# LepistaBioinformatics/blutils

Measured on AMD Instinct MI355X. Metric: Mqueries/sec consensus (synthetic outfmt-6 hit table), higher is better.
Workload: dtype i32/u32

## Files before the change

### blutils_amd/csrc/consensus_kernel.hip

```cpp

#if defined(__HIP_DEVICE_COMPILE__) && !defined(__gfx950__)
#error "consensus_kernel.hip is written for gfx950"
#endif

#include <hip/hip_runtime.h>

#include <climits>
#include <cstdint>
#include <type_traits>

#include "blu_internal.h"

namespace blu {

#define WAVE 64

constexpr int BLOCK_A = 768;
constexpr int BLU_WAVES_PER_SIMD = 3;
constexpr int BLOCK_N = 1024;
constexpr int BLU_N_WAVES_PER_SIMD = 4;
constexpr int BLOCK_F = 704;
constexpr int LIST_CAP = 208;
constexpr int LIST_CAP_RING = 248;
constexpr int LIST_CAP_F64 = 232;
// ... 681 lines not shown
                else { m[0] = wave_max_i32(m[0]); m[1] = wave_max_i32(m[1]); }
                uint32_t c[2], slot[2], tot[2], tmask[2];
#pragma unroll
                for (int hf = 0; hf < 2; ++hf) {
                    c[hf] = 0; tmask[hf] = 0;
#pragma unroll
                    for (int r = 0; r < 4; ++r) { const bool t = left[hf] > r && bs[hf][r] == m[hf]; tmask[hf] |= (uint32_t)t << r; c[hf] += (uint32_t)t; }
                    uint32_t in = c[hf];
                    in += (uint32_t)dpp<0x111>((int)in);
                    in += (uint32_t)dpp<0x112>((int)in);
                    in += (uint32_t)dpp<0x114>((int)in);
                    in += (uint32_t)dpp<0x118>((int)in);
                    const uint32_t k0 = (uint32_t)rl((int)in, 15), k1 = (uint32_t)rl((int)in, 31), k2 = (uint32_t)rl((int)in, 47), k3 = (uint32_t)rl((int)in, 63);
                    tot[hf] = k0 + k1 + k2 + k3;
                    slot[hf] = (row16 == 0 ? 0u : (row16 == 1 ? k0 : (row16 == 2 ? k0 + k1 : k0 + k1 + k2))) + in - c[hf];
                }
                const uint32_t gk = tot[0] + tot[1];
                const bool fits = fill + gk <= CAP;
                if (lane == 0) {
                    if (halves) L.meta[qi] = fits ? (fill | (gk << 16)) : META_SLOW;
                    else {
                        L.meta[qs[0]] = fits ? (fill | (tot[0] << 16)) : META_SLOW;
                        if (qs[1] < 64u) L.meta[qs[1]] = fits ? ((fill + tot[0]) | (tot[1] << 16)) : META_SLOW;
                    }
                }
                if (!fits) {
                    uint64_t rest = long_mask;
                    while (rest) { const uint32_t qn = (uint32_t)__builtin_ctzll(rest); rest &= rest - 1; if (lane == 0) L.meta[qn] = META_SLOW; }
                    break;
                }
                {
#pragma unroll
                    for (int hf = 0; hf < 2; ++hf) {
                        if (tot[hf] == 0) continue;
                        StepRegs S;
                        fetch_rest(S, voff[hf], tmask[hf]);
                        uint32_t idx = fill + (hf ? tot[0] : 0u) + slot[hf];
#pragma unroll
                        for (int r = 0; r < 4; ++r) {
                            if ((tmask[hf] >> r) & 1u) {
                                put_entry(idx, S, r, ro[hf] + sub4 + r);
                                ++idx;
                            }
                        }
                    }
                    fill += gk;
                }
            }
        };
        auto phase1_flat = [&]() {
            if constexpr (!RING) {
            constexpr uint32_t UR = FLAT_ROWS, MAXS = FLAT_STEPS, DEPTH = FLAT_DEPTH;
            static_assert(UR == 8u, "two 16-byte loads per lane");
            static_assert(FLAT_SEG >= MAX_TASK_SEG, "the flat pass takes every segment of the task");
            static_assert(DEPTH <= MAXS && MAXS * WAVE >= FLAT_SEG / UR, "a query's units fit one round");
            const uint32_t rows = L.seg[lane].y;
            const uint32_t nunit = (rows + UR - 1u) / UR;
            uint32_t incl = nunit;
            incl += (uint32_t)dpp<0x111>((int)incl);
            incl += (uint32_t)dpp<0x112>((int)incl);
            incl += (uint32_t)dpp<0x114>((int)incl);
            incl += (uint32_t)dpp<0x118>((int)incl);
            const uint32_t t0 = (uint32_t)rl((int)incl, 15), t1 = (uint32_t)rl((int)incl, 31), t2 = (uint32_t)rl((int)incl, 47);
            const uint32_t r16 = (uint32_t)lane >> 4;
            incl += r16 == 0 ? 0u : (r16 == 1 ? t0 : (r16 == 2 ? t0 + t1 : t0 + t1 + t2));
            const uint32_t q_end = incl, q_begin = incl - nunit;
            const uint64_t out_m = __ballot(rows != 0u && q_end > MAXS * WAVE);
            const uint32_t q_lim = out_m ? (uint32_t)__builtin_ctzll(out_m) : WAVE;
            const uint32_t total = q_lim < WAVE ? (uint32_t)rl((int)q_begin, (int)q_lim) : (uint32_t)rl((int)q_end, WAVE - 1);
            const uint32_t ns = (total + WAVE - 1u) / WAVE;
            L.qs[lane] = q_begin;
            L.qm[lane] = INT_MIN;
            L.qk[lane] = 0u;
            if (rows != 0u) L.meta[lane] = META_SLOW;
            __builtin_amdgcn_fence(__ATOMIC_RELEASE, "workgroup");
            __builtin_amdgcn_wave_barrier();
            __builtin_amdgcn_fence(__ATOMIC_ACQUIRE, "workgroup");
            auto issue = [&](const uint32_t st, u32x4& lo4, u32x4& hi4, uint32_t& um) {
                um = 0u;
                uint32_t voff = 0xFFFFFFF0u;
                int left = 0;
                if (st < ns) {
                    const uint32_t g = st * WAVE + (uint32_t)lane;
                    uint32_t q = 0;
#pragma unroll
                    for (uint32_t sp = 32; sp; sp >>= 1) { const uint32_t c = q + sp; if (L.qs[c] <= g) q = c; }
                    const uint2 sg = L.seg[q];
                    const uint32_t oq = g - L.qs[q];
                    left = g < total ? (int)sg.y - (int)(UR * oq) : 0;
                    if (left > 0) { voff = (sg.x + UR * oq) * 4u; um = q | (oq << 6) | (umin((uint32_t)left, UR) << 12); }
                }
                lo4 = __builtin_amdgcn_raw_buffer_load_b128(rs_bs, voff, 0, STREAM_AUX);
                hi4 = __builtin_amdgcn_raw_buffer_load_b128(rs_bs, left > 4 ? voff + 16u : 0xFFFFFFF0u, 0, STREAM_AUX);
            };
            u32x4 ba[DEPTH], bb[DEPTH];
            uint32_t um[MAXS];
            int lmx[MAXS];
#pragma unroll
            for (uint32_t st = 0; st < MAXS; ++st) { um[st] = 0u; lmx[st] = INT_MIN; }
#pragma unroll
            for (uint32_t st = 0; st < DEPTH; ++st) issue(st, ba[st], bb[st], um[st]);
#pragma unroll
            for (uint32_t st = 0; st < MAXS; ++st) {
                if (st >= ns) break;
                const u32x4 va = ba[st % DEPTH], vb = bb[st % DEPTH];
                const uint32_t left = (um[st] >> 12) & 15u;
                const uint32_t v[8] = {va.x, va.y, va.z, va.w, vb.x, vb.y, vb.z, vb.w};
                int bsv[UR], mx = INT_MIN;
#pragma unroll
                for (uint32_t r = 0; r < UR; ++r) { bsv[r] = left > r ? (int)v[r] : INT_MIN; mx = imax(mx, bsv[r]); }
                uint32_t lmask = 0;
#pragma unroll
                for (uint32_t r = 0; r < UR; ++r) lmask |= (uint32_t)(left > r && bsv[r] == mx) << r;
                um[st] |= lmask << 16;
                lmx[st] = mx;
                if (left) atomicMax(&L.qm[um[st] & 63u], mx);
                if (st + DEPTH < MAXS) issue(st + DEPTH, ba[st % DEPTH], bb[st % DEPTH], um[st + DEPTH]);
            }
            __builtin_amdgcn_fence(__ATOMIC_RELEASE, "workgroup");
            __builtin_amdgcn_wave_barrier();
            __builtin_amdgcn_fence(__ATOMIC_ACQUIRE, "workgroup");
            uint32_t running = fill, q_cut = q_lim;
#pragma unroll
            for (uint32_t st = 0; st < MAXS; ++st) {
                if (st >= ns) break;
                const uint32_t q = um[st] & 63u, oq = (um[st] >> 6) & 63u;
                const bool have = ((um[st] >> 12) & 15u) != 0u;
                const int M = L.qm[q];
                const uint32_t tmask = (have && lmx[st] == M) ? (um[st] >> 16) & 0xFFu : 0u;
                const uint32_t c = (uint32_t)__builtin_popcount(tmask);
                uint32_t in2 = c;
                in2 += (uint32_t)dpp<0x111>((int)in2);
                in2 += (uint32_t)dpp<0x112>((int)in2);
                in2 += (uint32_t)dpp<0x114>((int)in2);
                in2 += (uint32_t)dpp<0x118>((int)in2);
                const uint32_t k0 = (uint32_t)rl((int)in2, 15), k1 = (uint32_t)rl((int)in2, 31), k2 = (uint32_t)rl((int)in2, 47), k3 = (uint32_t)rl((int)in2, 63);
                in2 += r16 == 0 ? 0u : (r16 == 1 ? k0 : (r16 == 2 ? k0 + k1 : k0 + k1 + k2));
                const uint32_t idx0 = running + in2 - c;
                if (have && oq == 0u) L.meta[q] = META_SLOW | idx0;
                if (c) atomicAdd(&L.qk[q], c);
                const bool over = have && idx0 + c > CAP;
                const uint64_t over_m = __ballot(over);
                const bool room = !over && c != 0u && (over_m == 0ull || (uint32_t)lane < (uint32_t)__builtin_ctzll(over_m));
                if (room) L.rec[idx0] = make_uint4(__builtin_bitreverse32(tmask), L.seg[q].x + UR * oq, UR * oq, 0u);
                if (over_m) { q_cut = (uint32_t)rl((int)q, __builtin_ctzll(over_m)); break; }
                running += k0 + k1 + k2 + k3;
            }
            __builtin_amdgcn_fence(__ATOMIC_RELEASE, "workgroup");
            __builtin_amdgcn_wave_barrier();
            __builtin_amdgcn_fence(__ATOMIC_ACQUIRE, "workgroup");
            const uint32_t m = L.meta[lane];
            if (rows != 0u && (uint32_t)lane < q_cut) L.meta[lane] = (m & 0xFFFFu) | (L.qk[lane] << 16);
            fill = q_cut < q_lim ? (L.meta[q_cut] & 0xFFFFu) : running;
            if (q_cut < WAVE) stop_q = q_cut;
            }
        };
        auto ring_mark_landed = [&](const uint32_t upto) {
            const uint32_t m0 = (ring_landed + RING_CHUNKS - 1u) & ~(RING_CHUNKS - 1u);
            if (m0 < upto) {
                if ((uint32_t)lane < RING_PAD) L.ring[RING_ROWS + lane] = L.ring[lane];
                __builtin_amdgcn_fence(__ATOMIC_RELEASE, "workgroup");
                __builtin_amdgcn_wave_barrier();
                __builtin_amdgcn_fence(__ATOMIC_ACQUIRE, "workgroup");
            }
            ring_landed = upto;
        };
        auto ring_refill = [&]() {
            if (ring_head < ring_tail) { ring_head = ring_tail; if (ring_landed < ring_tail) ring_landed = ring_tail; }
            const uint32_t lim = ring_end < ring_tail + RING_CHUNKS ? ring_end : ring_tail + RING_CHUNKS;
            if (ring_head < lim) { ring_dma_run(rs_ring, ring_c0, ring_head, lim); ring_head = lim; }
        };
        auto phase1_scan = [&](const auto rpl_c, const auto full_c, const uint32_t LPQ) {
            constexpr uint32_t RPL = decltype(rpl_c)::value;
            constexpr bool FULL = decltype(full_c)::value;
            static_assert(RPL <= RING_PAD && RPL <= 32u, "rows per lane");
            const uint32_t QPS = WAVE / LPQ;
            const uint32_t grp = (uint32_t)lane / LPQ, sub = ((uint32_t)lane & (LPQ - 1u)) * RPL, row16 = (uint32_t)lane >> 4;
            {
                const uint32_t cs = (uint32_t)((vbase + (uint32_t)rl((int)seg_x, (int)first_q)) >> 8);
                if (cs < ring_tail) { wait_vmcnt(0u); ring_head = ring_landed = ring_tail = cs; }
            }
            for (uint32_t qb = first_q / QPS * QPS; qb < nq; qb += QPS) {
                const uint32_t r_lo = (uint32_t)rl((int)seg_x, (int)(qb < first_q ? first_q : qb));
                const uint32_t qn = qb + QPS;
                const uint32_t r_hi = qn < nq ? (uint32_t)rl((int)seg_x, (int)qn) : task_nrows;
                ring_tail = (uint32_t)((vbase + r_lo) >> 8);
                ring_refill();
                if (r_hi > r_lo) {
                    const uint32_t need = (uint32_t)((vbase + r_hi - 1u) >> 8);
                    if (need >= ring_landed) { wait_vmcnt(ring_head - 1u - need); ring_mark_landed(need + 1u); }
                }
                const uint32_t qi = qb + grp;
                const uint2 sg = L.seg[qi];
                const int left0 = (sg.y > short_seg ? 0 : (int)sg.y) - (int)sub;
                const uint32_t over = (FULL && left0 > 0 && left0 < (int)RPL) ? RPL - (uint32_t)left0 : 0u;
                const uint32_t sub_e = sub - over;
                const int left = FULL ? (left0 > 0 ? (int)RPL : 0) : left0;
                const uint32_t row0 = sg.x + sub_e;
                const uint32_t a = ((uint32_t)vbase + sg.x + sub_e) & RING_MASK;
                int b[RPL];
#pragma unroll
                for (uint32_t i = 0; i < RPL; ++i) b[i] = (int)L.ring[a + i];
                asm volatile("s_waitcnt lgkmcnt(0)" ::: "memory");
#pragma unroll
                for (uint32_t i = 0; i < RPL; ++i) asm volatile("" : "+v"(b[i]));
                if (r_hi > r_lo) { ring_tail = (uint32_t)((vbase + r_hi) >> 8); ring_refill(); }
                int M = INT_MIN;
                if constexpr (FULL) {
#pragma unroll
                    for (uint32_t i = 0; i < RPL; ++i) M = imax(M, b[i]);
                    M = left > 0 ? M : INT_MIN;
                } else {
#pragma unroll
                    for (uint32_t i = 0; i < RPL; ++i) { b[i] = (int)i < left ? b[i] : INT_MIN; M = imax(M, b[i]); }
                }
                if (LPQ >= 2) M = imax(M, dpp<0xB1>(M));
                if (LPQ >= 4) M = imax(M, dpp<0x4E>(M));
                if (LPQ >= 8) M = imax(M, dpp<0x141>(M));
                if (LPQ >= 16) M = imax(M, dpp<0x140>(M));
                uint32_t mask = tie_mask<RPL>(b, M);
                mask = left > 0 ? mask : 0u;
                if constexpr (FULL) mask &= 0xFFFFFFFFu >> (32u - RPL + over);
                const uint32_t c = (uint32_t)__builtin_popcount(mask);
                uint32_t incl = c;
                incl += (uint32_t)dpp<0x111>((int)incl);
                incl += (uint32_t)dpp<0x112>((int)incl);
                incl += (uint32_t)dpp<0x114>((int)incl);
                incl += (uint32_t)dpp<0x118>((int)incl);
                const uint32_t k0 = (uint32_t)rl((int)incl, 15), k1 = (uint32_t)rl((int)incl, 31);
                const uint32_t k2 = (uint32_t)rl((int)incl, 47), k3 = (uint32_t)rl((int)incl, 63);
                const bool fits = fill + k0 + k1 + k2 + k3 <= CAP;
                const uint32_t p1 = fill + k0, p2 = p1 + k1, p3 = p2 + k2;
                const uint32_t rbase = row16 == 0 ? fill : (row16 == 1 ? p1 : (row16 == 2 ? p2 : p3));
                uint32_t gk = c;
                if (LPQ >= 2) gk += (uint32_t)dpp<0xB1>((int)gk);
                if (LPQ >= 4) gk += (uint32_t)dpp<0x4E>((int)gk);
                if (LPQ >= 8) gk += (uint32_t)dpp<0x141>((int)gk);
                if (LPQ >= 16) gk += (uint32_t)dpp<0x140>((int)gk);
                if (PID32 && !fits) {
                    __builtin_amdgcn_s_setprio(2);
                    uint64_t BK = 0;
                    uint32_t bacc = 0, bpos = 0, brow = 0, kmin = 0xFFFFFFFFu, pmax = 0, dlo = 0xFFFFFFFFu, dhi = 0, err = 0xFFFFFFFFu;
                    auto reset = [&]() { BK = 0; bacc = 0; bpos = 0; brow = 0; kmin = 0xFFFFFFFFu; pmax = 0; dlo = 0xFFFFFFFFu; dhi = 0; err = 0xFFFFFFFFu; };
                    auto better = [&](const uint64_t K, const uint32_t acc, const uint32_t pos, const uint64_t K2, const uint32_t acc2, const uint32_t pos2) {
                        const bool gt = (K > K2) | ((K == K2) & (acc > acc2)), eq = (K == K2) & (acc == acc2);
                        return STRAT == BLU_RELAXED ? (gt | (eq & (pos > pos2))) : ((!gt & !eq) | (eq & (pos < pos2)));
                    };
                    auto take_record = [&](const u32x4 rec, const uint32_t gp, const bool on) {
                        const uint32_t len = umin(rec.x >> BLU_ROW_BITS, t.max_depth), pos = rec.x & ROW_MASK;
                        const bool unmatched = pos >= t.n_tax, bad = !unmatched && (rec.x >> BLU_ROW_BITS) == 0;
                        const uint32_t e = (gp << 8) | (bad ? (uint32_t)BLU_ST_ERR_BAD_LINEAGE : (uint32_t)BLU_ST_ERR_UNMATCHED_TAXID);
                        err = (on && (unmatched | bad)) ? umin(err, e) : err;
                        const uint32_t pm = rec.y & ((1u << KEY_PID_BITS) - 1u);
                        const uint32_t k1 = (len << KEY_PID_BITS) | pm;
                        const uint64_t K = ((uint64_t)k1 << 32) | (rec.z ^ 0x80000000u);
                        const bool take = on & ((kmin == 0xFFFFFFFFu) | better(K, rec.w, gp, BK, bacc, bpos));
                        BK = take ? K : BK; bacc = take ? rec.w : bacc; bpos = take ? gp : bpos; brow = take ? pos : brow;
                        kmin = on ? umin(kmin, k1) : kmin;
                        const uint32_t pmo = pm | ((!PACKED && rec.y >= (1u << KEY_PID_BITS)) ? 0x80000000u : 0u);
                        pmax = (on && pmo > pmax) ? pmo : pmax;
                        dlo = on ? umin(dlo, pos) : dlo;
                        dhi = (on && pos > dhi) ? pos : dhi;
                    };
                    auto load_record = [&](const uint32_t row, const bool on) {
                        u32x4 r;
                        if (PACKED) r = __builtin_amdgcn_raw_buffer_load_b128(rs_tax, on ? row * 16u : 0xFFFFFFC0u, 0, GATHER_AUX);
                        else {
                            const uint32_t o4 = on ? row * 4u : 0xFFFFFFF0u;
                            r.x = __builtin_amdgcn_raw_buffer_load_b32(rs_tax, o4, 0, GATHER_AUX);
                            r.y = __builtin_amdgcn_raw_buffer_load_b32(rs_pid, o4, 0, GATHER_AUX);
                            r.z = __builtin_amdgcn_raw_buffer_load_b32(rs_aln, o4, 0, GATHER_AUX);
                            r.w = __builtin_amdgcn_raw_buffer_load_b32(rs_acc, o4, 0, GATHER_AUX);
                        }
                        return r;
                    };
                    auto merge = [&](auto ctrl) {
                        constexpr int C = decltype(ctrl)::value;
                        const uint64_t K2 = ((uint64_t)(uint32_t)dpp<C>((int)(uint32_t)(BK >> 32)) << 32) | (uint32_t)dpp<C>((int)(uint32_t)BK);
                        const uint32_t acc2 = (uint32_t)dpp<C>((int)bacc), pos2 = (uint32_t)dpp<C>((int)bpos), row2 = (uint32_t)dpp<C>((int)brow);
                        const uint32_t kmin2 = (uint32_t)dpp<C>((int)kmin);
                        const bool take = (kmin2 != 0xFFFFFFFFu) & ((kmin == 0xFFFFFFFFu) | better(K2, acc2, pos2, BK, bacc, bpos));
                        BK = take ? K2 : BK; bacc = take ? acc2 : bacc; bpos = take ? pos2 : bpos; brow = take ? row2 : brow;
                        kmin = umin(kmin, kmin2);
                        const uint32_t pm2 = (uint32_t)dpp<C>((int)pmax); pmax = pm2 > pmax ? pm2 : pmax;
                        dlo = umin(dlo, (uint32_t)dpp<C>((int)dlo));
                        const uint32_t hi2 = (uint32_t)dpp<C>((int)dhi); dhi = hi2 > dhi ? hi2 : dhi;
                        err = umin(err, (uint32_t)dpp<C>((int)err));
                    };
                    auto deliver = [&](const int src, const bool mine) {
                        const uint32_t f_khi = (uint32_t)__builtin_amdgcn_ds_bpermute(src, (int)(uint32_t)(BK >> 32));
                        const uint32_t f_pos = (uint32_t)__builtin_amdgcn_ds_bpermute(src, (int)bpos), f_row = (uint32_t)__builtin_amdgcn_ds_bpermute(src, (int)brow);
                        const uint32_t f_kmin = (uint32_t)__builtin_amdgcn_ds_bpermute(src, (int)kmin), f_pmax = (uint32_t)__builtin_amdgcn_ds_bpermute(src, (int)pmax);
                        const uint32_t f_lo = (uint32_t)__builtin_amdgcn_ds_bpermute(src, (int)dlo), f_hi = (uint32_t)__builtin_amdgcn_ds_bpermute(src, (int)dhi);
                        const uint32_t f_err = (uint32_t)__builtin_amdgcn_ds_bpermute(src, (int)err);
                        const bool got = mine && f_kmin != 0xFFFFFFFFu;
                        const bool g_ovf = got && (f_pmax & 0x80000000u) != 0u, g_err = got && !g_ovf && f_err != 0xFFFFFFFFu, g_ok = got && !g_ovf && !g_err;
                        dn_flag = g_ovf ? 3u : (g_err ? 2u : (g_ok ? 1u : dn_flag));
                        dn_err = g_err ? (f_err & 0xFFu) : dn_err;
                        dn_pos = g_err ? (f_err >> 8) : dn_pos;
                        if constexpr (PID32) { r_pid = g_ok ? (f_khi & ((1u << KEY_PID_BITS) - 1u)) : r_pid; max_pid = g_ok ? f_pmax : max_pid; }
                        r_len = g_ok ? (f_khi >> KEY_PID_BITS) : r_len; r_row = g_ok ? f_row : r_row; r_pos = g_ok ? f_pos : r_pos;
                        minlen = g_ok ? (f_kmin >> KEY_PID_BITS) : minlen; g_lo = g_ok ? f_lo : g_lo; g_hi = g_ok ? f_hi : g_hi;
                    };
                    const uint32_t tq = (uint32_t)lane;
                    const bool mine = tq >= qb && tq < qn && tq < nq;
                    const uint32_t own0 = (mine ? tq - qb : 0u) * LPQ;
                    if (LPQ <= 4u && BLU_DENSE_Q * (k0 + k1 + k2 + k3) >= r_hi - r_lo) {
                        const uint32_t c4 = (uint32_t)lane & 3u;
#pragma nounroll
                        for (uint32_t g = 0; g < 4u; ++g) {
                            const int own = (int)((16u * g + ((uint32_t)lane >> 2)) * 4u);
                            const uint32_t o_row0 = (uint32_t)__builtin_amdgcn_ds_bpermute(own, (int)row0);
                            const uint32_t o_mask = (uint32_t)__builtin_amdgcn_ds_bpermute(own, (int)mask);
                            const uint32_t o_sub = (uint32_t)__builtin_amdgcn_ds_bpermute(own, (int)sub_e);
                            if (__ballot(o_mask != 0u) == 0ull) continue;
                            reset();
                            constexpr uint32_t NF = PACKED ? 4u : 2u;
#pragma unroll
                            for (uint32_t b0 = 0; b0 < RPL; b0 += 4u * NF) {
                                if (__ballot(((o_mask >> (RPL - 4u * NF - b0)) & ((1u << (4u * NF)) - 1u)) != 0u) == 0ull) continue;
                                u32x4 rq[NF];
#pragma unroll
                                for (uint32_t j = 0; j < NF; ++j) {
                                    const uint32_t i = b0 + 4u * j + c4;
                                    rq[j] = load_record(o_row0 + i, ((o_mask >> (RPL - 1u - i)) & 1u) != 0u);
                                }
#pragma unroll
                                for (uint32_t j = 0; j < NF; ++j) {
                                    const uint32_t i = b0 + 4u * j + c4;
                                    take_record(rq[j], o_sub + i, ((o_mask >> (RPL - 1u - i)) & 1u) != 0u);
                                }
                            }
                            merge(std::integral_constant<int, 0xB1>());
                            merge(std::integral_constant<int, 0x4E>());
                            if (LPQ >= 2) merge(std::integral_constant<int, 0x141>());
                            if (LPQ >= 4) merge(std::integral_constant<int, 0x140>());
                            deliver((int)(((own0 & 15u) * 4u) * 4u), mine && (own0 >> 4) == g);
                        }
                    } else {
                        uint32_t m = mask;
                        while (__ballot(m != 0u)) {
                            u32x4 rq[4];
                            uint32_t gp[4];
#pragma unroll
                            for (int j = 0; j < 4; ++j) {
                                const bool on = m != 0u;
                                const uint32_t hb = on ? 31u - (uint32_t)__builtin_clz(m) : 0u, i = RPL - 1u - hb;
                                m = on ? (m & ~(1u << hb)) : 0u;
                                gp[j] = on ? sub_e + i : 0xFFFFFFFFu;
                                rq[j] = load_record(row0 + i, on);
                            }
#pragma unroll
                            for (int j = 0; j < 4; ++j) take_record(rq[j], gp[j], gp[j] != 0xFFFFFFFFu);
                        }
                        if (LPQ >= 2) merge(std::integral_constant<int, 0xB1>());
                        if (LPQ >= 4) merge(std::integral_constant<int, 0x4E>());
                        if (LPQ >= 8) merge(std::integral_constant<int, 0x141>());
                        if (LPQ >= 16) merge(std::integral_constant<int, 0x140>());
                        deliver((int)(own0 * 4u), mine);
                    }
                    {
                        const uint32_t f_gk = (uint32_t)__builtin_amdgcn_ds_bpermute((int)(own0 * 4u), (int)gk);
                        dn_k = (mine && dn_flag == 1u) ? f_gk : dn_k;
                    }
                    if (sub == 0 && gk != 0u) L.meta[qi] = META_DENSE;
                    __builtin_amdgcn_s_setprio(0);
                    continue;
                }
                uint32_t idx = rbase + incl - c;
                if (!fits) {
                    const uint32_t lane_o = (uint32_t)__builtin_ctzll(__ballot(idx + c > CAP));
                    const uint32_t qo = qb + lane_o / LPQ;
                    const bool taken = qi < qo;
                    if (sub == 0) L.meta[qi] = taken ? (idx | (gk << 16)) : META_SLOW;
                    if (taken && c) { L.rec[idx].x = mask << (32u - RPL); L.rec[idx].y = DESC_WORD1(RPL, row0, sub_e); }
                    fill = (uint32_t)rl((int)idx, (int)((qo - qb) * LPQ));
                    stop_q = qo;
                    wait_vmcnt(0u);
                    ring_head = ring_landed = ring_tail = (uint32_t)((vbase + (uint32_t)rl((int)seg_x, (int)qo)) >> 8);
                    break;
                }
                if (sub == 0) L.meta[qi] = idx | (gk << 16);
                fill = p3 + k3;
                static_assert((RPL == 16u || RPL == 32u) && SHORT_SEG <= 128u, "descriptor word of a lane");
                if (c) { L.rec[idx].x = mask << (32u - RPL); L.rec[idx].y = DESC_WORD1(RPL, row0, sub_e); }
            }
        };
        auto gather_list = [&](auto&& between) {
            constexpr int NG = (CAP + WAVE - 1) / WAVE;
            u32x4 g[NG];
            uint32_t ghi[NG], gpos[NG], ghint[NG];
            uint32_t carry = 0;
#pragma unroll
            for (int u = 0; u < NG; ++u) {
                g[u] = u32x4{0u, 0u, 0u, 0u}; ghi[u] = 0u; gpos[u] = 0u; ghint[u] = 0u;
                if ((uint32_t)u * WAVE >= fill_ring) continue;
                const uint32_t idx = (uint32_t)u * WAVE + (uint32_t)lane;
                const bool valid = idx < fill_ring;
                const uint32_t d0 = L.rec[idx < CAP ? idx : 0u].x;
                int s = (valid && d0 != 0u) ? (int)idx : 0;
                s = imax(s, dpp<0x111>(s));
                s = imax(s, dpp<0x112>(s));
                s = imax(s, dpp<0x114>(s));
                s = imax(s, dpp<0x118>(s));
                s = imax(s, __builtin_amdgcn_update_dpp(0, s, 0x142, 0xA, 0xF, false));
                s = imax(s, __builtin_amdgcn_update_dpp(0, s, 0x143, 0xC, 0xF, false));
                s = imax(s, (int)carry);
                carry = (uint32_t)rl(s, 63);
                const uint4 dd = L.rec[s];
                const uint32_t d0w = dd.x, d = dd.y;
                uint32_t r = idx - (uint32_t)s, x = scan_rpl == 32u ? d0w : d0w >> 16, i = 0;
                if (scan_rpl == 32u) {
                    const uint32_t h = x >> 16, ch = (uint32_t)__builtin_popcount(h);
                    const bool low = r >= ch;
                    r -= low ? ch : 0u; x = low ? (x & 0xFFFFu) : h; i += low ? 16u : 0u;
                }
                {
                    const uint32_t h = x >> 8, ch = (uint32_t)__builtin_popcount(h);
                    const bool low = r >= ch;
                    r -= low ? ch : 0u; x = low ? (x & 0xFFu) : h; i += low ? 8u : 0u;
                }
                {
                    const uint32_t h = x >> 4, ch = (uint32_t)__builtin_popcount(h);
                    const bool low = r >= ch;
                    r -= low ? ch : 0u; x = low ? (x & 0xFu) : h; i += low ? 4u : 0u;
                }
                {
                    const uint32_t h = x >> 2, ch = (uint32_t)__builtin_popcount(h);
                    const bool low = r >= ch;
                    r -= low ? ch : 0u; x = low ? (x & 0x3u) : h; i += low ? 2u : 0u;
                }
                i += (r >= (x >> 1)) ? 1u : 0u;
                const uint32_t row = (RING ? (d >> DESC_SUB_BITS) : d) + i;
                gpos[u] = (RING ? (d & ((1u << DESC_SUB_BITS) - 1u)) : dd.z) + i;
                if (PACKED) g[u] = __builtin_amdgcn_raw_buffer_load_b128(rs_tax, valid ? row * 16u : 0xFFFFFFC0u, 0, GATHER_AUX);
                else if (WIDE) {
                    g[u] = __builtin_amdgcn_raw_buffer_load_b128(rs_tax, valid ? row * 24u : 0xFFFFFFC0u, 0, GATHER_AUX);
                    const u32x2 p = __builtin_amdgcn_raw_buffer_load_b64(rs_tax, valid ? row * 24u + 16u : 0xFFFFFFE0u, 0, GATHER_AUX);
                    ghint[u] = g[u].y;
                    g[u].y = p.x; ghi[u] = p.y;
                } else {
                    const uint32_t o4 = valid ? row * 4u : 0xFFFFFFF0u;
                    g[u].x = __builtin_amdgcn_raw_buffer_load_b32(rs_tax, o4, 0, GATHER_AUX);
                    if (PID32) g[u].y = __builtin_amdgcn_raw_buffer_load_b32(rs_pid, o4, 0, GATHER_AUX);
                    else {
                        const u32x2 p = __builtin_amdgcn_raw_buffer_load_b64(rs_pid, valid ? row * 8u : 0xFFFFFFE0u, 0, GATHER_AUX);
                        g[u].y = p.x; ghi[u] = p.y;
                    }
                    g[u].z = __builtin_amdgcn_raw_buffer_load_b32(rs_aln, o4, 0, GATHER_AUX);
                    g[u].w = __builtin_amdgcn_raw_buffer_load_b32(rs_acc, o4, 0, GATHER_AUX);
                }
            }
            between();
            bool ovf = false;
            uint32_t gk[NG];
#pragma unroll
            for (int u = 0; u < NG; ++u) {
                const bool valid = (uint32_t)u * WAVE + (uint32_t)lane < fill_ring;
                if constexpr (PID32) { gk[u] = g[u].y & PM_MASK; ovf |= !PACKED && valid && g[u].y >= (1u << KEY_PID_BITS); }
                else {
                    const double p = __hiloint2double((int)ghi[u], (int)g[u].y);
                    const bool in_range = p >= 0.0 && p < 131.0705;
                    const uint32_t k = in_range ? (uint32_t)(p * 1000.0 + 0.5) : 0u;
                    const double back = milli17_to_f64(k);
                    gk[u] = k;
                    ovf |= valid && !(in_range && __double2hiint(back) == (int)ghi[u] && __double2loint(back) == (int)g[u].y && k < BLU_KTHR_NEVER);
                }
            }
            keyed = __ballot(ovf) == 0ull && fill == fill_ring;
            bool any_bad = false;
#pragma unroll
            for (int u = 0; u < NG; ++u) {
                const uint32_t idx = (uint32_t)u * WAVE + (uint32_t)lane;
                if (idx < fill_ring) {
                    if (keyed) {
                        const uint32_t len = umin(g[u].x >> BLU_ROW_BITS, t.max_depth);
                        any_bad |= len == 0u || (g[u].x & ROW_MASK) >= t.n_tax;
                        const uint32_t hint = (PID32 ? g[u].y : ghint[u]) >> KEY_PID_BITS;
                        L.rec[idx] = make_uint4((g[u].x & ROW_MASK) | ((hint >> 8) << BLU_ROW_BITS),
                                                (len << KEYED_LEN_SHIFT) | (gk[u] << KEYED_PID_SHIFT) | (hint & 0xFFu), g[u].z ^ 0x80000000u, g[u].w);
                    } else L.rec[idx] = make_uint4(g[u].x, g[u].y, g[u].z, g[u].w);
                    L.pq[idx] = (uint16_t)gpos[u];
                    if (!PID32) L.p1[idx] = ghi[u];
                }
            }
            keyed_bad = __ballot(any_bad) != 0ull;
        };
        bool pend = (uint32_t)lane < nq;
        uint32_t pend_before = WAVE + 1;
        if (RING && contiguous) {
            ring_c0 = (uint32_t)(vbase >> 8);
            rs_ring = ring_desc(ring_c0);
            ring_end = task_nrows ? (uint32_t)((vbase + task_nrows - 1u) >> 8) + 1u : ring_c0;
            if (pref_q0 != q0_32) ring_head = ring_landed = ring_c0;
            ring_tail = ring_c0;
        }
        for (;;) {
        fill = 0;
        stop_q = WAVE;
        bool ring_round = false;
        bool list_round = false;
        keyed = false;
        {
            const uint32_t rows = L.seg[lane].y;
            const uint64_t live = __ballot(rows != 0u);
            first_q = live ? (uint32_t)__builtin_ctzll(live) : 0u;
            {
                const uint32_t n16 = (uint32_t)__builtin_popcountll(__ballot(rows != 0u && rows <= 16u));
                const uint32_t n32 = (uint32_t)__builtin_popcountll(__ballot(rows != 0u && rows <= 32u));
                const uint32_t n64 = (uint32_t)__builtin_popcountll(__ballot(rows != 0u && rows <= 64u));
                const uint32_t n128 = (uint32_t)__builtin_popcountll(__ballot(rows != 0u && rows <= SHORT_SEG));
                const uint32_t c16 = 4u * n16 + BLU_LONG_COST * (n128 - n16), c32 = 8u * n32 + BLU_LONG_COST * (n128 - n32);
                const uint32_t c64 = 16u * n64 + BLU_LONG_COST * (n128 - n64), c128 = 32u * n128;
                uint32_t best = c128;
                short_seg = SHORT_SEG;
                if (c64 < best) { best = c64; short_seg = 64u; }
                if (c32 < best) { best = c32; short_seg = 32u; }
                if (c16 < best) { best = c16; short_seg = 16u; }
            }
            bool flat_round = false;
            if constexpr (!RING) {
                const uint32_t n128 = (uint32_t)__builtin_popcountll(__ballot(rows != 0u && rows <= SHORT_SEG));
                const uint32_t n_over = (uint32_t)__builtin_popcountll(__ballot(rows > SHORT_SEG));
                uint32_t best;
                {
                    const uint32_t n16 = (uint32_t)__builtin_popcountll(__ballot(rows != 0u && rows <= 16u));
                    const uint32_t n32 = (uint32_t)__builtin_popcountll(__ballot(rows != 0u && rows <= 32u));
                    const uint32_t n64 = (uint32_t)__builtin_popcountll(__ballot(rows != 0u && rows <= 64u));
                    best = 32u * n128;
                    best = umin(best, 16u * n64 + BLU_LONG_COST * (n128 - n64));
                    best = umin(best, 8u * n32 + BLU_LONG_COST * (n128 - n32));
                    best = umin(best, 4u * n16 + BLU_LONG_COST * (n128 - n16));
                }
                const uint32_t units = (uint32_t)wave_sum_u32((rows + FLAT_ROWS - 1u) / FLAT_ROWS);
                flat_round = units != 0u && units + units / 4u + 64u < best + BLU_LONG_COST * n_over;
                if (flat_round) { short_seg = FLAT_SEG; scan_rpl = 16u; }
            }
            const uint32_t longest = flat_round ? 0u : wave_max_u32(rows > short_seg ? 0u : rows);
            ring_round = RING && contiguous && longest != 0u && all_short && __ballot(rows > short_seg) == 0ull;
            uint32_t lpq = 1;
            if (ring_round) {
                scan_rpl = longest > 32u ? 32u : 16u;
                while (lpq * scan_rpl < longest) lpq *= 2;
                while ((WAVE / lpq) * longest + 256u > RING_ROWS) lpq *= 2;
            }
            list_round = ring_round || flat_round;
            if (list_round) {
#pragma unroll
                for (uint32_t u = 0; u * WAVE < CAP; ++u) { const uint32_t i = u * WAVE + (uint32_t)lane; if (i < CAP) L.rec[i].x = 0u; }
            }
            if (ring_round) {
                const bool all_full = __ballot(rows != 0u && rows <= short_seg && rows < scan_rpl) == 0ull;
                if (scan_rpl == 32u) {
                    if (all_full) phase1_scan(std::integral_constant<uint32_t, 32>(), std::true_type(), lpq);
                    else phase1_scan(std::integral_constant<uint32_t, 32>(), std::false_type(), lpq);
                } else phase1_scan(std::integral_constant<uint32_t, 16>(), std::false_type(), lpq);
            }
            else if (flat_round) phase1_flat();
            else if (longest > 32u && longest <= 64u) phase1(std::integral_constant<uint32_t, 16>(), false);
            else if (longest) phase1(longest <= 16u ? 4u : (longest <= 32u ? 8u : 32u), longest >= (PACKED ? 9u : 25u));
            if (stop_q < WAVE && rows != 0u && ((uint32_t)lane >= stop_q || rows > short_seg)) L.meta[lane] = META_SLOW;
            fill_ring = list_round ? fill : 0u;
            const uint64_t long_mask = __ballot(rows > short_seg);
            if (long_mask && stop_q == WAVE) phase1_long(long_mask);
        }
        __builtin_amdgcn_fence(__ATOMIC_RELEASE, "workgroup");
        __builtin_amdgcn_wave_barrier();
        __builtin_amdgcn_fence(__ATOMIC_ACQUIRE, "workgroup");
        const bool last_round = __ballot(pend && (my_end - my_off) != 0u && (my_end - my_off) <= MAX_TASK_SEG && in_span && (L.meta[lane] & META_SLOW)) == 0ull;
        uint32_t nxt_c0 = 0, nxt_lim = 0;
        if (RING && last_round && nx_nq != 0u) {
            uint32_t n_off = nx_off, n_end = nx_end;
            asm volatile("" : "+v"(n_off), "+v"(n_end));
            if (n_end > n_hits32) n_end = n_hits32;
            if (n_off > n_end) n_off = n_end;
            const uint32_t nqn = nx_nq;
            const uint32_t n_start = (uint32_t)rl((int)n_off, 0);
            const bool n_span = n_off >= n_start && (n_end - n_start) <= (uint32_t)TASK_SPAN;
            const uint32_t rel_end = n_end - n_start, rel_off = n_off - n_start;
            const uint32_t prev_end = (uint32_t)__shfl_up((int)rel_end, 1);
            const bool ok = n_span && (n_end - n_off) <= SHORT_SEG && (lane == 0 || rel_off == prev_end);
            const uint32_t n_rows = (uint32_t)rl((int)rel_end, (int)nqn - 1);
            if (__ballot((uint32_t)lane < nqn && !ok) == 0ull && n_rows != 0u) {
                const uint64_t vb = (uint64_t)n_start + mis;
                nxt_c0 = (uint32_t)(vb >> 8);
                const uint32_t cend = (uint32_t)((vb + n_rows - 1u) >> 8) + 1u;
                nxt_lim = cend < nxt_c0 + RING_CHUNKS ? cend : nxt_c0 + RING_CHUNKS;
            }
        }
        auto prefetch_next = [&]() {
            if (nxt_lim > nxt_c0) {
                const auto rsn = ring_desc(nxt_c0);
                ring_dma_run(rsn, nxt_c0, nxt_c0, nxt_lim);
                ring_head = nxt_lim; ring_landed = nxt_c0; ring_tail = nxt_c0;
                pref_q0 = nx_q0;
            }
        };
        __builtin_amdgcn_s_setprio(3);
        if (list_round) gather_list(prefetch_next);
        else prefetch_next();
        __builtin_amdgcn_fence(__ATOMIC_RELEASE, "workgroup");
        __builtin_amdgcn_wave_barrier();
        __builtin_amdgcn_fence(__ATOMIC_ACQUIRE, "workgroup");

        {
            const uint32_t nrows = my_end - my_off;
            const uint32_t m = L.meta[lane];
            const bool listed = pend && nrows != 0 && nrows <= MAX_TASK_SEG && in_span && !(m & (META_SLOW | META_DENSE));
            const uint32_t first = listed ? (m & 0xFFFFu) : 0u, k = listed ? ((m >> 16) & 0x3FFu) : 0u;
            const uint32_t kmax = wave_max_u32(k);
            uint32_t err = 0, err_pos = 0, nan_pos = 0xFFFFFFFFu;
            uint32_t b_len = 0, b_acc = 0, lo = 0xFFFFFFFFu, hi = 0, l_minlen = 0xFFFFFFFFu, l_row = 0, l_pos = 0, l_hint = 0;
            int b_aln = 0;
            PK b_pid = 0, l_maxpid = 0;
            const uint32_t last_e = k ? k - 1u : 0u;
            uint4 nx_rec = make_uint4(0, 0, 0, 0);
            uint32_t nx_pq = 0;
            uint32_t l_keyed = 0;
            if (!keyed) { nx_rec = L.rec[first]; nx_pq = L.pq[first]; }
            if (keyed) {
                l_keyed = 1u;
                uint64_t BK = 0;
                uint32_t kmin = 0xFFFFFFFFu, pmax = 0;
                uint32_t l_idx = first;
                auto step = [&](const auto check_c, const uint4 x, const uint32_t xidx, const bool is_first) {
                    const uint32_t pos = x.x & ROW_MASK;
                    if constexpr (decltype(check_c)::value) {
                        const bool unmatched = pos >= t.n_tax, bad = x.y < (1u << KEYED_LEN_SHIFT);
                        const bool first_err = (err == 0) & (unmatched | bad);
                        err = first_err ? (unmatched ? (uint32_t)BLU_ST_ERR_UNMATCHED_TAXID : (uint32_t)BLU_ST_ERR_BAD_LINEAGE) : err;
                        err_pos = first_err ? (uint32_t)L.pq[xidx] : err_pos;
                    }
                    kmin = umin(kmin, x.y);
                    lo = umin(lo, pos);
                    hi = pos > hi ? pos : hi;
                    const uint32_t ky = x.y & ~0xFFu;
                    const uint32_t pm = (x.y >> KEYED_PID_SHIFT) & PM_MASK;
                    pmax = pm > pmax ? pm : pmax;
                    const uint64_t K = ((uint64_t)ky << 32) | x.z;
                    const bool gt = (K > BK) | ((K == BK) & (x.w > b_acc)), eq = (K == BK) & (x.w == b_acc);
                    const bool take = is_first | (STRAT == BLU_RELAXED ? (gt | eq) : !(gt | eq));
                    BK = take ? K : BK;
                    b_acc = take ? x.w : b_acc;
                    l_idx = take ? xidx : l_idx;
                };
                auto reduce = [&](const auto check_c) {
                    for (uint32_t e = 0; e < kmax; e += 4) {
                        uint4 x[4];
                        uint32_t xi[4];
#pragma unroll
                        for (uint32_t j = 0; j < 4; ++j) {
                            xi[j] = first + (e + j < k ? e + j : last_e);
                            x[j] = L.rec[xi[j]];
                        }
#pragma unroll
                        for (uint32_t j = 0; j < 4; ++j) step(check_c, x[j], xi[j], e == 0 && j == 0);
                    }
                };
                if (keyed_bad) reduce(std::true_type()); else reduce(std::false_type());
                const uint32_t l_x = L.rec[l_idx].x, l_y = L.rec[l_idx].y;
                l_pos = L.pq[l_idx];
                const uint32_t k1 = (uint32_t)(BK >> 32);
                b_len = k1 >> KEYED_LEN_SHIFT;
                l_minlen = kmin >> KEYED_LEN_SHIFT;
                l_row = l_x & ROW_MASK;
                l_hint = ((l_x >> BLU_ROW_BITS) << 8) | (l_y & 0xFFu);
                if constexpr (PID32) { b_pid = (k1 >> KEYED_PID_SHIFT) & PM_MASK; l_maxpid = pmax; }
                else { b_pid = milli17_to_f64((k1 >> KEYED_PID_SHIFT) & PM_MASK); l_maxpid = milli17_to_f64(pmax); }
            } else {
                for (uint32_t e = 0; e < kmax; ++e) {
                    const uint4 x = nx_rec;
                    const uint32_t xpos = nx_pq;
                    const uint32_t idx = first + (e < k ? e : last_e), idn = first + (e + 1u < k ? e + 1u : last_e);
                    nx_rec = L.rec[idn];
                    nx_pq = L.pq[idn];
                    const uint32_t len = umin(x.x >> BLU_ROW_BITS, t.max_depth), pos = x.x & ROW_MASK;
                    const bool unmatched = pos >= t.n_tax, bad = (x.x >> BLU_ROW_BITS) == 0;
                    const bool first_err = (err == 0) & (unmatched | bad);
                    err = first_err ? (unmatched ? (uint32_t)BLU_ST_ERR_UNMATCHED_TAXID : (uint32_t)BLU_ST_ERR_BAD_LINEAGE) : err;
                    err_pos = first_err ? xpos : err_pos;
                    PK xpid;
                    if constexpr (PID32) xpid = PACKED ? (x.y & PM_MASK) : x.y;
                    else {
                        xpid = __hiloint2double((int)L.p1[idx], (int)x.y);
                        nan_pos = (nan_pos == 0xFFFFFFFFu && xpid != xpid) ? xpos : nan_pos;
                    }
                    l_minlen = umin(l_minlen, len);
                    lo = umin(lo, pos);
                    hi = pos > hi ? pos : hi;
                    l_maxpid = xpid > l_maxpid ? xpid : l_maxpid;
                    const bool take = (e == 0) | key_better<STRAT, PK>(len, xpid, (int)x.z, x.w, b_len, b_pid, b_aln, b_acc);
                    b_len = take ? len : b_len;
                    b_pid = take ? xpid : b_pid;
                    b_aln = take ? (int)x.z : b_aln;
                    b_acc = take ? x.w : b_acc;
                    l_row = take ? pos : l_row;
                    l_pos = take ? xpos : l_pos;
                    if (PACKED) l_hint = take ? (x.y >> KEY_PID_BITS) : l_hint;
                }
            }
            if (pend) {
                bool done = true;
                if (nrows == 0) { st_code = BLU_ST_NO_HITS; st_ref = 0xFFFFFFFFu; rec_kind = 2; }
                else if (nrows > MAX_TASK_SEG || !in_span) wl_push(wl_q, wl_cnt, (uint32_t)q);
                else if (m & META_SLOW) done = false;
                else if (dn_flag == 1) mode = dn_k == 1 ? 2u : 0u;
                else if (dn_flag == 2) { st_code = dn_err; st_ref = row0 + dn_pos; rec_kind = 2; }
                else if (dn_flag == 3) wl_push(wl_q, wl_cnt, (uint32_t)q);
                else if (err) { st_code = err; st_ref = row0 + err_pos; rec_kind = 2; }
                else if (!PID32 && nan_pos != 0xFFFFFFFFu) { st_code = BLU_ST_ERR_BAD_PIDENT; st_ref = row0 + nan_pos; rec_kind = 2; }
                else {
                    r_len = b_len | (l_hint << 8) | (l_keyed << 30); r_pid = b_pid; r_row = l_row; r_pos = l_pos; minlen = l_minlen; max_pid = l_maxpid;
                    mode = k == 1 ? 2u : 0u;
                    g_lo = lo; g_hi = hi;
                }
                if (done) { pend = false; L.seg[lane].y = 0u; }
            }
        }
        const uint32_t pend_now = (uint32_t)__builtin_popcountll(__ballot(pend));
        if (pend_now == 0 || pend_now >= pend_before) break;
        pend_before = pend_now;
        __builtin_amdgcn_fence(__ATOMIC_RELEASE, "workgroup");
        __builtin_amdgcn_wave_barrier();
        __builtin_amdgcn_fence(__ATOMIC_ACQUIRE, "workgroup");
        }
        if (pend) wl_push(wl_q, wl_cnt, (uint32_t)q);

        if (mode != 3) {
            const bool single = mode == 2;
            rec_kind = 1;
            const uint32_t r_hint = (r_len >> 8) & ((1u << BLU_HINT_BITS) - 1u);
            const bool r_keyed = (r_len >> 30) != 0u;
            r_len &= 0xFFu;
            const bool spread = !single && g_lo < g_hi;
            const uint32_t dl = r_row - g_lo, dh = g_hi - r_row;
            const bool wide = spread && (dl > BLU_ROW_RUN_MAX || dh > BLU_ROW_RUN_MAX);
            const bool wide_tab = wide && t.wblk != nullptr;
            uint2 wentry = make_uint2(0u, 0u);
            if (wide_tab) wentry = t.wblk[g_lo >> BLU_WBLK_SHIFT];
            const uint32_t* ref = t.lin + (uint64_t)r_row * t.stride;
            const uint4* ref4 = reinterpret_cast<const uint4*>(ref);
            constexpr bool NODE_RELOAD = LAYOUT == 1 || LAYOUT == 3 || !RING || STRAT == BLU_CAUTIOUS;
            constexpr uint32_t NID_REGS = NODE_RELOAD ? 0u : 12u;
            static_assert(NID_REGS <= 20u, "a 128-byte row holds 20 node ids");
            uint4 w[8];
#pragma unroll
            for (int k = 0; k < (NODE_RELOAD ? 3 : (int)((BLU_ROW_NODE_BASE + NID_REGS + 3u) / 4u)); ++k) w[k] = ref4[k];
            uint4 ck[4] = {};
            uint32_t shape_req = 0xFFFFFFFFu;
            if constexpr (PACKED || WIDE) {
                if (r_hint) {
                    shape_req = umin(r_hint - 1u, t.n_shapes - 1u);
                    const uint4* kg = reinterpret_cast<const uint4*>(t.kthr + (uint64_t)shape_req * t.cstride);
#pragma unroll
                    for (int k = 0; k < 4; ++k) ck[k] = kg[k];
                }
            }
            uint32_t d_tab = 0;
            if (wide_tab) {
                const uint32_t wn = wide_node(wentry, g_lo);
                const uint4* ch = reinterpret_cast<const uint4*>(t.wchain + (uint64_t)(wn == 0xFFFFFFFFu ? 0u : wn) * BLU_WCHAIN);
                const uint4 c0 = ch[0], c1 = ch[1], c2 = ch[2];
                d_tab = chain_count4(c0, g_hi) + chain_count4(c1, g_hi) + chain_count4(c2, g_hi);
                if (t.wide_levels > BLU_WCHAIN_FIRST && d_tab == BLU_WCHAIN_FIRST) {
                    d_tab += chain_count4(ch[3], g_hi);
                    if (t.wide_levels > BLU_WCHAIN && d_tab == BLU_WCHAIN) {
                        const uint4* cg = reinterpret_cast<const uint4*>(t.wchain_hi + (uint64_t)wn * BLU_WCHAIN);
                        d_tab += chain_count4(cg[0], g_hi) + chain_count4(cg[1], g_hi) + chain_count4(cg[2], g_hi) + chain_count4(cg[3], g_hi);
                    }
                }
                if (wn == 0xFFFFFFFFu) d_tab = shared_levels(t, g_lo, g_hi);
            } else if (wide) d_tab = shared_levels(t, g_lo, g_hi);
            __builtin_amdgcn_s_setprio(1);
            r_hdr = w[0].x;
            const uint32_t len_ref = umin(r_len, r_hdr & 0xFF);
            d = minlen;
            if (wide) d = umin(minlen, d_tab);
            else if (spread) {
                const uint32_t ca = dl * 0x01010101u, cb = dh * 0x01010101u, H = 0x80808080u;
                uint32_t cnt = 0;
                cnt += (uint32_t)__builtin_popcount((w[0].y - ca) & (w[1].z - cb) & H);
                cnt += (uint32_t)__builtin_popcount((w[0].z - ca) & (w[1].w - cb) & H);
                cnt += (uint32_t)__builtin_popcount((w[0].w - ca) & (w[2].x - cb) & H);
                cnt += (uint32_t)__builtin_popcount((w[1].x - ca) & (w[2].y - cb) & H);
                cnt += (uint32_t)__builtin_popcount((w[1].y - ca) & (w[2].z - cb) & H);
                if (cnt >= BLU_ROW_IV_LEVELS && minlen > BLU_ROW_IV_LEVELS) d = umin(minlen, shared_levels(t, g_lo, g_hi));
                else d = umin(minlen, cnt);
            }
            const bool agree = single | (d >= minlen);
            if (!agree && d == 0) { st_code = BLU_ST_ERR_ROOT_DISAGREE; st_ref = row0 + r_pos; rec_kind = 2; }
            else {
                const uint32_t shape = umin(r_hdr >> 8, t.n_shapes - 1u);
                const uint32_t* codes = t.codes + (uint64_t)shape * t.cstride;
                const uint4* codes4 = reinterpret_cast<const uint4*>(codes);
                const uint32_t* lvl = t.kthr + (uint64_t)shape * t.cstride;
                const uint4* lvl4 = reinterpret_cast<const uint4*>(lvl);
                const uint32_t b = single ? len_ref : (agree ? minlen - 1 : d - 1);
                double ident;
                if constexpr (PACKED) ident = milli17_to_f64(((single | agree) ? r_pid : max_pid) & PM_MASK);
                else ident = pid_f64<PID32>((single | agree) ? r_pid : max_pid);
// ... 577 lines not shown
```

Measured before the change: 11610.

## Double-buffer record loads across batches and owner groups in dense consensus path

Restructures the dense consensus inner loop into a software pipeline. The record loads for the next batch, or for the next owner group, are issued before the current batch is consumed, using two alternating register buffers. Row, sub-index and gk are packed into one word so each owner needs one fewer bpermute. The sparse path gets the same ping-pong prefetch. In exchange, register pressure rises from the double buffers, and the packing assumes row0 fits in 16 bits and sub_e and gk in 8 bits.

```diff
diff --git a/blutils_amd/csrc/consensus_kernel.hip b/blutils_amd/csrc/consensus_kernel.hip
--- a/blutils_amd/csrc/consensus_kernel.hip
+++ b/blutils_amd/csrc/consensus_kernel.hip
@@ -1007,56 +1007,101 @@
                         r_len = g_ok ? (f_khi >> KEY_PID_BITS) : r_len; r_row = g_ok ? f_row : r_row; r_pos = g_ok ? f_pos : r_pos;
                         minlen = g_ok ? (f_kmin >> KEY_PID_BITS) : minlen; g_lo = g_ok ? f_lo : g_lo; g_hi = g_ok ? f_hi : g_hi;
                     };
+                    const uint32_t my_rs = (row0 & 0xFFFFu) | (sub_e << 16) | (gk << 24);
                     const uint32_t tq = (uint32_t)lane;
                     const bool mine = tq >= qb && tq < qn && tq < nq;
                     const uint32_t own0 = (mine ? tq - qb : 0u) * LPQ;
                     if (LPQ <= 4u && BLU_DENSE_Q * (k0 + k1 + k2 + k3) >= r_hi - r_lo) {
                         const uint32_t c4 = (uint32_t)lane & 3u;
+                        constexpr uint32_t NF = PACKED ? 4u : 2u;
+                        constexpr uint32_t NB = RPL / (4u * NF);
+                        struct Owner { uint32_t rs, mask; };
+                        auto owner_of = [&](const uint32_t g) {
+                            const int own = (int)((16u * (g & 3u) + ((uint32_t)lane >> 2)) * 4u);
+                            Owner o;
+                            o.rs = (uint32_t)__builtin_amdgcn_ds_bpermute(own, (int)my_rs);
+                            o.mask = (uint32_t)__builtin_amdgcn_ds_bpermute(own, (int)mask);
+                            o.mask = g < 4u ? o.mask : 0u;
+                            return o;
+                        };
+                        auto issue = [&](u32x4 (&rq)[NF], const Owner& o, const uint32_t b0) {
+#pragma unroll
+                            for (uint32_t j = 0; j < NF; ++j) {
+                                const uint32_t i = b0 + 4u * j + c4;
+                                rq[j] = load_record((o.rs & 0xFFFFu) + i, ((o.mask >> (RPL - 1u - i)) & 1u) != 0u);
+                            }
+                        };
+                        auto take = [&](const u32x4 (&rq)[NF], const Owner& o, const uint32_t b0) {
+                            if (__ballot(((o.mask >> (RPL - 4u * NF - b0)) & ((1u << (4u * NF)) - 1u)) != 0u) == 0ull) return;
+#pragma unroll
+                            for (uint32_t j = 0; j < NF; ++j) {
+                                const uint32_t i = b0 + 4u * j + c4;
+                                take_record(rq[j], ((o.rs >> 16) & 0xFFu) + i, ((o.mask >> (RPL - 1u - i)) & 1u) != 0u);
+                            }
+                        };
+                        Owner cur = owner_of(0u);
+                        u32x4 ra[NF], rb[NF];
+                        issue(ra, cur, 0u);
+                        auto group = [&](const uint32_t g, const Owner cur, u32x4 (&r0)[NF], u32x4 (&r1)[NF]) {
+                            const Owner nxt = owner_of(g + 1u);
+                            const bool any = __ballot(cur.mask != 0u) != 0ull;
+                            reset();
+                            auto batch = [&](auto bi_c, u32x4 (&have)[NF], u32x4 (&next)[NF]) {
+                                constexpr uint32_t bi = decltype(bi_c)::value;
+                                if constexpr (bi + 1u < NB) issue(next, cur, (bi + 1u) * 4u * NF);
+                                else issue(next, nxt, 0u);
+                                take(have, cur, bi * 4u * NF);
+                            };
+                            batch(std::integral_constant<uint32_t, 0>(), r0, r1);
+                            if constexpr (NB >= 2u) batch(std::integral_constant<uint32_t, 1>(), r1, r0);
+                            if constexpr (NB >= 4u) { batch(std::integral_constant<uint32_t, 2>(), r0, r1); batch(std::integral_constant<uint32_t, 3>(), r1, r0); }
+                            static_assert(NB == 1u || NB == 2u || NB == 4u, "batches of an owner group");
+                            if (any) {
+                                merge(std::integral_constant<int, 0xB1>());
+                                merge(std::integral_constant<int, 0x4E>());
+                                if (LPQ >= 2) merge(std::integral_constant<int, 0x141>());
+                                if (LPQ >= 4) merge(std::integral_constant<int, 0x140>());
+                                deliver((int)(((own0 & 15u) * 4u) * 4u), mine && (own0 >> 4) == g);
+                            }
+                            return nxt;
+                        };
 #pragma nounroll
-                        for (uint32_t g = 0; g < 4u; ++g) {
-                            const int own = (int)((16u * g + ((uint32_t)lane >> 2)) * 4u);
-                            const uint32_t o_row0 = (uint32_t)__builtin_amdgcn_ds_bpermute(own, (int)row0);
-                            const uint32_t o_mask = (uint32_t)__builtin_amdgcn_ds_bpermute(own, (int)mask);
-                            const uint32_t o_sub = (uint32_t)__builtin_amdgcn_ds_bpermute(own, (int)sub_e);
-                            if (__ballot(o_mask != 0u) == 0ull) continue;
-                            reset();
-                            constexpr uint32_t NF = PACKED ? 4u : 2u;
-#pragma unroll
-                            for (uint32_t b0 = 0; b0 < RPL; b0 += 4u * NF) {
-                                if (__ballot(((o_mask >> (RPL - 4u * NF - b0)) & ((1u << (4u * NF)) - 1u)) != 0u) == 0ull) continue;
-                                u32x4 rq[NF];
-#pragma unroll
-                                for (uint32_t j = 0; j < NF; ++j) {
-                                    const uint32_t i = b0 + 4u * j + c4;
-                                    rq[j] = load_record(o_row0 + i, ((o_mask >> (RPL - 1u - i)) & 1u) != 0u);
-                                }
-#pragma unroll
-                                for (uint32_t j = 0; j < NF; ++j) {
-                                    const uint32_t i = b0 + 4u * j + c4;
-                                    take_record(rq[j], o_sub + i, ((o_mask >> (RPL - 1u - i)) & 1u) != 0u);
-                                }
-                            }
-                            merge(std::integral_constant<int, 0xB1>());
-                            merge(std::integral_constant<int, 0x4E>());
-                            if (LPQ >= 2) merge(std::integral_constant<int, 0x141>());
-                            if (LPQ >= 4) merge(std::integral_constant<int, 0x140>());
-                            deliver((int)(((own0 & 15u) * 4u) * 4u), mine && (own0 >> 4) == g);
+                        for (uint32_t g = 0; g < 4u; g += (NB & 1u) ? 2u : 1u) {
+                            cur = group(g, cur, ra, rb);
+                            if constexpr ((NB & 1u) != 0u) cur = group(g + 1u, cur, rb, ra);
                         }
                     } else {
                         uint32_t m = mask;
-                        while (__ballot(m != 0u)) {
-                            u32x4 rq[4];
-                            uint32_t gp[4];
+                        auto pick = [&](u32x4 (&rq)[4], uint32_t& rows4) {
+                            rows4 = 0u;
 #pragma unroll
                             for (int j = 0; j < 4; ++j) {
                                 const bool on = m != 0u;
                                 const uint32_t hb = on ? 31u - (uint32_t)__builtin_clz(m) : 0u, i = RPL - 1u - hb;
                                 m = on ? (m & ~(1u << hb)) : 0u;
-                                gp[j] = on ? sub_e + i : 0xFFFFFFFFu;
+                                rows4 |= (on ? i : 0xFFu) << (8 * j);
                                 rq[j] = load_record(row0 + i, on);
                             }
-#pragma unroll
-                            for (int j = 0; j < 4; ++j) take_record(rq[j], gp[j], gp[j] != 0xFFFFFFFFu);
+                        };
+                        auto take4 = [&](const u32x4 (&rq)[4], const uint32_t rows4) {
+#pragma unroll
+                            for (int j = 0; j < 4; ++j) {
+                                const uint32_t i = (rows4 >> (8 * j)) & 0xFFu;
+                                take_record(rq[j], sub_e + i, i != 0xFFu);
+                            }
+                        };
+                        u32x4 ra[4], rb[4];
+                        uint32_t pa, pb;
+                        pick(ra, pa);
+                        for (;;) {
+                            const bool more_b = __ballot(m != 0u) != 0ull;
+                            pick(rb, pb);
+                            take4(ra, pa);
+                            if (!more_b) break;
+                            const bool more_a = __ballot(m != 0u) != 0ull;
+                            pick(ra, pa);
+                            take4(rb, pb);
+                            if (!more_a) break;
                         }
                         if (LPQ >= 2) merge(std::integral_constant<int, 0xB1>());
                         if (LPQ >= 4) merge(std::integral_constant<int, 0x4E>());
@@ -1065,10 +1110,10 @@
                         deliver((int)(own0 * 4u), mine);
                     }
                     {
-                        const uint32_t f_gk = (uint32_t)__builtin_amdgcn_ds_bpermute((int)(own0 * 4u), (int)gk);
+                        const uint32_t f_gk = (uint32_t)__builtin_amdgcn_ds_bpermute((int)(own0 * 4u), (int)my_rs) >> 24;
                         dn_k = (mine && dn_flag == 1u) ? f_gk : dn_k;
                     }
-                    if (sub == 0 && gk != 0u) L.meta[qi] = META_DENSE;
+                    if (sub == 0 && (my_rs >> 24) != 0u) L.meta[qi] = META_DENSE;
                     __builtin_amdgcn_s_setprio(0);
                     continue;
                 }
@@ -1201,6 +1246,7 @@
             ring_tail = ring_c0;
         }
         for (;;) {
+        if constexpr (RING && PID32) asm volatile("" : "+v"(lane));
         fill = 0;
         stop_q = WAVE;
         bool ring_round = false;
```

After: 11590. No clear change (-0.2%).
